# ReactiveBayes/Cortex.jl

Hardware: AMD Instinct MI355X
Metric: edge-message updates/sec per sweep, 10M-edge Gaussian grid (higher is better)
Workload: dtype f64; 1 GPU; C4: ONE 1415x1415 2-D Gaussian grid loopy BP; 10005465 bipartite edges, 16006480 owned directed message updates + 2002225 marginals per sweep; whole job 16006480 updates per sweep; schedule=fused, partition=1 row blocks, seed=1234

## Files before the change

### cortex.jl_amd/_lib.py

```python
from __future__ import annotations

import ctypes as C
import os

HERE = os.path.dirname(os.path.abspath(__file__))
LIB_PATH = os.environ.get("CORTEX_HIP_LIB", os.path.join(HERE, "libcortex_hip.so"))

ABI_VERSION = 9
OK = 0
ERR_INVALID_ARGUMENT, ERR_NOT_FOUND, ERR_UNSUPPORTED, ERR_STATE, ERR_DEVICE, ERR_NO_DEVICE, ERR_OUT_OF_MEMORY = (
    -1, -2, -3, -4, -5, -6, -7)
TO_FACTOR, TO_VARIABLE = 1, 2
ITEM_MESSAGE_TO_FACTOR, ITEM_MESSAGE_TO_VARIABLE, ITEM_INDIVIDUAL_MARGINAL = 1, 2, 4
ITEM_PRODUCT_OF_MESSAGES, ITEM_JOINT_MARGINAL = 8, 16
FORM_MOMENT, FORM_POINT, FORM_NATURAL, FORM_MEAN_PRECISION, FORM_GAMMA = 0, 1, 2, 3, 4
FACTOR_OPAQUE, FACTOR_GAUSS_ADDITIVE, FACTOR_GAUSS_LINEAR, FACTOR_NORMAL_PRECISION, FACTOR_BERNOULLI, FACTOR_GAUSS_LINEAR_N = 0, 1, 2, 3, 4, 5
NPARAM = 4
ROLE_OUT, ROLE_IN, ROLE_PRECISION = 0, 1, 2
SCHED_FLOODING, SCHED_FUSED, SCHED_CHAIN_SCAN, SCHED_TREE, SCHED_REFERENCE = 0, 1, 2, 3, 4
FAMILY_GAUSSIAN, FAMILY_NATURAL2, FAMILY_VMP_MEAN_FIELD, FAMILY_VMP_STRUCTURED = 0, 1, 2, 3
VMP_ALL_NORMAL, VMP_ALL_PRECISION = -1, -2
WIRE_WEAK, WIRE_INTERMEDIATE, WIRE_NO_LISTEN, WIRE_DEFAULT_VARIABLE, WIRE_LINK = 1, 2, 4, 8, 16
KERNEL_VAR_TO_FACTOR, KERNEL_FACTOR_TO_VAR, KERNEL_FUSED, KERNEL_BATCH, KERNEL_BIG_VAR = 0, 1, 2, 3, 4
KERNEL_HALO_BEGIN, KERNEL_HALO_END = 5, 6
# ... 52 lines not shown
    "cx_ref_trace": (_i32, [_vp, _i64, C.POINTER(Item), _pi64]),
    "cx_residual": (_i32, [_vp, _pd]),
    "cx_message_health": (_i32, [_vp, _pi64]),
    "cx_log_evidence": (_i32, [_vp, _pd, _pi64]),
    "cx_graph_components": (_i32, [_vp, _i64, _pi64, _pi64, _pi64]),
    "cx_log_evidence_components": (_i32, [_vp, _i64, _pd, _pi64, _pi64, _pi64]),
    "cx_log_evidence_mfma": (_i32, [_vp, _pd, _pi64]),
    "cx_factor_beliefs": (_i32, [_vp, _i64, _pi64, _pd]),
    "cx_factor_statistics": (_i32, [_vp, _i64, _pi64, _pi64, _i64, _pd, _pi64]),
    "cx_factor_beliefs_mfma": (_i32, [_vp, _i64, _pi64, _pd]),
    "cx_factor_statistics_mfma": (_i32, [_vp, _i64, _pi64, _pi64, _i64, _pd, _pi64]),
    "cx_sample_posterior": (_i32, [_vp, _i64, C.c_uint64, _pd, _i64, _pi64, _pd, _pi64]),
    "cx_linear_moments": (_i32, [_vp, _i64, _pi64, _pi64, _pd, _pd, _pd, _pi64]),
    "cx_predictive": (_i32, [_vp, _i32, _i64, _pi64, _pd, _pd, _pi64]),
    "cx_predictive_rows": (_i32, [_vp, _i64, _pi64, _pi64]),
    "cx_predictive_mfma": (_i32, [_vp, _i32, _i64, _pi64, _pd, _pd, _pi64]),
    "cx_predictive_rows_mfma": (_i32, [_vp, _i64, _pi64, _pi64]),
    "cx_causal_marginals": (_i32, [_vp, _i32, _i32, _i64, _pi64, _pd, _pi64]),
    "cx_causal_marginals_mfma": (_i32, [_vp, _i32, _i32, _i64, _pi64, _pd, _pi64]),
    "cx_sample_posterior_mfma": (_i32, [_vp, _i64, C.c_uint64, _pd, _i64, _pi64, _pd, _pi64]),
    "cx_set_factor_offsets": (_i32, [_vp, _i64, _pi64, _pd]),
    "cx_halo_configure": (_i32, [_vp, _i64, _pi64, _pi64, _i64, _pi64, _pi64]),
    "cx_halo_buffers": (_i32, [_vp, C.POINTER(_vp), _pi64, C.POINTER(_vp), _pi64]),
    "cx_halo_set_buffers": (_i32, [_vp, _vp, _vp]),
    "cx_sweep_begin": (_i32, [_vp]),
    "cx_sweep_main": (_i32, [_vp]),
    "cx_sweep_end": (_i32, [_vp]),
    "cx_comm_unique_id": (_i32, [_vp]),
    "cx_comm_init": (_i32, [_vp, _i32, _i32, _vp]),
    "cx_halo_peers": (_i32, [_vp, _i32, _pi32, _pi64, _pi64, _pi64, _pi64]),
    "cx_sweep_exchange": (_i32, [_vp, _i32]),
    "cx_sweep_until": (_i32, [_vp, _dbl, _i32, _i32, _pi32, _pd]),
    "cx_halo_configure_state": (_i32, [_vp, _i64, _pi64, _pi64, _i64, _pi64, _pi64]),
    "cx_halo_set_layers": (_i32, [_vp, _i64, _pi64, _pi32, _i32]),
    "cx_halo_state_pack": (_i32, [_vp]),
    "cx_halo_state_unpack": (_i32, [_vp]),
    "cx_halo_state_exchange": (_i32, [_vp]),
    "cx_halo_exchange_sweep": (_i32, [_vp, _i32]),
    "cx_halo_ipc_alloc": (_i32, [_vp, C.c_char_p, C.POINTER(C.c_void_p), _pi64]),
    "cx_halo_ipc_connect": (_i32, [_vp, _i32, C.c_char_p, C.c_void_p, _i32, _i64, _i64]),
    "cx_halo_ipc_exchange": (_i32, [_vp]),
    "cx_halo_ipc_exchange_sweep": (_i32, [_vp, _i32]),
    "cx_halo_ipc_batch": (_i32, [_vp, _i32]),
    "cx_halo_ipc_set_fused": (_i32, [_vp, _i32]),
    "cx_halo_ipc_push": (_i32, [_vp]),
    "cx_halo_ipc_unpack": (_i32, [_vp]),
    "cx_halo_ipc_status": (_i32, [_vp, _pi32, _pi64]),
    "cx_halo_ipc_set_timeout": (_i32, [_vp, C.c_double]),
    "cx_chain_block_maps": (_i32, [_vp, _pd, _pd, _pd, _pd, _pi64, _pi64, _pi64]),
    "cx_chain_plan_stats": (_i32, [_vp, _pi64]),
    "cx_chain_scan_stats": (_i32, [_vp, _pi64]),
    "cx_sweep_stats": (_i32, [_vp, _pi64]),
    "cx_sweep_deep_stats": (_i32, [_vp, _pi64]),
    "cx_tree_plan_stats": (_i32, [_vp, _pi64]),
    "cx_tree_heavy_path_stats": (_i32, [_vp, _pi64]),
    "cx_set_marginals": (_i32, [_vp, _i64, _pi64, _i32, _pd]),
    "cx_update_marginals": (_i32, [_vp, _i64, _pi64]),
    "cx_state_bytes": (_i32, [_vp, _pi64]),
    "cx_state_export": (_i32, [_vp, _vp, C.c_int64]),
    "cx_state_import": (_i32, [_vp, _vp, C.c_int64]),
    "cx_profile_enable": (_i32, [_vp, _i32]),
    "cx_profile_read": (_i32, [_vp, _i32, _pd, _pi64]),
    "cx_kernel_name": (C.c_char_p, [_i32]),
}

def item_range(lo: int, hi: int) -> int:
    return (int(lo) << 32) | int(hi)


_lib = None


class CortexHipError(RuntimeError):

    def __init__(self, code: int, message: str):
        super().__init__(f"cortex_hip status {code}: {message}")
        self.code = code
        self.message = message


def load():
    global _lib
    if _lib is not None:
        return _lib
    if not os.path.exists(LIB_PATH):
        raise ImportError(
            f"{LIB_PATH} is missing: build it with `python -m cortex.jl_amd.build` (hipcc --offload-arch=gfx950); "
            "there is no CPU fallback for the device path")
    lib = C.CDLL(LIB_PATH)
    for name, (res, args) in SIGNATURES.items():
        fn = getattr(lib, name)
        fn.restype = res
        fn.argtypes = args
    if lib.cx_version() != ABI_VERSION:
        raise ImportError(f"libcortex_hip.so ABI {lib.cx_version()} != binding ABI {ABI_VERSION}")
    _lib = lib
    return lib
```

### cortex.jl_amd/csrc/cx_api_sweep.hip

```cpp

#include "cx_host.h"
#include "cx_chains.h"
#include "cx_tree_plan.h"
#include "cx_lattice_deep.h"

using namespace cxh;

namespace cxh {

int32_t ensure_v2f(cx_handle *h) {
    if (!h->v2f_stale) return CX_OK;
    const double2 *src = h->d_f2v_alt ? h->d_f2v_alt : h->d_f2v;
    cx::launch_var_to_factor(h, src, false);
    cx::launch_big_var_to_factor(h, src, false);
    CX_HIP(h, hipGetLastError());
    h->v2f_stale = false;
    return CX_OK;
}

int32_t build_chains(cx_handle *h) {
    if (!h->chains_dirty) return CX_OK;
    if (h->cfg.dim > 1) { int32_t rc0 = mv_ensure_chain_msgs(h); if (rc0 != CX_OK) return rc0; }
    try {
        cx::chains::Out co;
// ... 243 lines not shown
                if (pi >= 0) (void)cx::chain64_tree_sweep(h, pi);
            } else if (kind == 0) {
                if (idx == h->tree_hp_marginal_stage && h->cfg.compute_marginals_in_sweep == 0) continue;
                const int64_t n = h->tree_stage_off[idx + 1] - h->tree_stage_off[idx];
                if (n > 0 && h->cfg.dim > 1) cx::mv_launch_batch(h, h->d_tree_rec + 5 * h->tree_stage_off[idx], n);
                else if (n > 0) cx::launch_batch(h, h->d_tree_rec + 5 * h->tree_stage_off[idx], n);
            } else if (h->cfg.dim > 1) {
                const int64_t l0 = h->tree_hp_link_off[idx];
                cx::mvc_launch_scan_range(h, h->tree_hp_npos, h->tree_hp_pos_off[idx + 1], l0, h->tree_hp_link_off[idx + 1] - l0, h->tree_hp_K[idx],
                                          kind == 1 ? h->d_chain_skip1 : h->d_tree_skip1_down, kind == 2);
            } else if (kind == 3) {
                const int64_t l0 = h->tree_hp_link_off[idx];
                cx::launch_kary_link_params(h, l0, h->tree_hp_link_off[idx + 1] - l0, h->d_tree_a ? h->d_tree_a : h->d_a, h->d_tree_b ? h->d_tree_b : h->d_b);
            } else {
                const int64_t p0 = h->tree_hp_pos_off[idx], l0 = h->tree_hp_link_off[idx];
                cx::launch_chain_scan_range(h, h->d_f2v, p0, h->tree_hp_pos_off[idx + 1] - p0, l0, h->tree_hp_link_off[idx + 1] - l0,
                                            kind == 1 ? h->d_chain_skip1 : h->d_tree_skip1_down, kind == 2);
            }
        }
        return;
    }
    size_t ns = h->tree_stage_off.empty() ? 0 : h->tree_stage_off.size() - 1;
    if (ns > 0 && h->cfg.compute_marginals_in_sweep == 0 && !cx::is_mfma_dim(h->cfg.dim)) ns--;
    static const bool runs = [] { const char *e = std::getenv("CX_TREE_RUNS"); return !(e && e[0] == '0'); }();
    for (size_t s = 0; s < ns;) {
        const int64_t n = h->tree_stage_off[s + 1] - h->tree_stage_off[s], nk = h->tree_kary_off[s + 1] - h->tree_kary_off[s];
        if (cx::is_mfma_dim(h->cfg.dim)) {
            const int64_t np = h->tree_pre_off[s + 1] - h->tree_pre_off[s];
            if (np > 0) cx::mv64_launch_v2f(h, (int)np, h->d_tree_pre_slots + h->tree_pre_off[s], h->d_tree_pre_vars + h->tree_pre_off[s], h->d_mv_f2v);
            if (n > 0) cx::mv64_launch_rule(h, (int)n, h->d_tree_rec + 8 * h->tree_stage_off[s], h->d_mv_f2v, h->d_mv_f2v, CX_KERNEL_BATCH);
            s++; continue;
        }
        if (h->cfg.dim > 1) { if (n > 0) cx::mv_launch_batch(h, h->d_tree_rec + 5 * h->tree_stage_off[s], n); s++; continue; }
        size_t e = s;
        while (runs && e < ns && h->tree_stage_off[e + 1] - h->tree_stage_off[e] <= 1024) e++;
        if (e >= s + 2) { cx::launch_batch_run(h, h->d_tree_rec, h->d_tree_stage_off, (int)s, (int)e); s = e; continue; }
        if (n > 0) cx::launch_batch(h, h->d_tree_rec + 5 * h->tree_stage_off[s], n);
        if (nk > 0) cx::launch_kary_items(h, h->d_tree_kary + h->tree_kary_off[s], nk);
        s++;
    }
}

int32_t tree_sweep(cx_handle *h) {
    static const bool graphs = [] { const char *e = std::getenv("CX_TREE_GRAPH"); return !(e && e[0] == '0'); }();
    cx::GraphExec &g = h->tree_graph;
    if (graphs && !h->profiling) {
        if (!g && !g.failed()) (void)capture(h, g, [h] { tree_issue(h); });
        if (g && launch(h, g)) return CX_OK;
    }
    tree_issue(h);
    return CX_OK;
}

constexpr int kDeepMax = 4, kDeepDefault = 4, kDeepMinSweeps = 16;
static int deep_depth_of_call(int32_t n_sweeps) {
    if (n_sweeps < kDeepMinSweeps) return 2;
    const char *e = std::getenv("CX_SWEEP_DEPTH");
    const int d = e ? std::atoi(e) : kDeepDefault;
    return d >= 2 && d <= kDeepMax ? d : kDeepDefault;
}

static int32_t pairs_allowed(cx_handle *h, int32_t n_sweeps, bool last_marg_only, bool *yes) {
    *yes = false;
    const char *e = std::getenv("CX_SWEEP_PAIRS");
    if (e && e[0] == '0') return CX_OK;
    if (n_sweeps < 3 || h->pair_H == 0 || h->cfg.dim != 1 || h->cfg.family != CX_FAMILY_GAUSSIAN || h->cfg.schedule != CX_SCHED_FUSED) return CX_OK;
    if (h->damping != 0.0 || h->any_linear || h->n_kary > 0 || !h->big_vars.empty() || h->halo_state || !h->recv_slots.empty() || !h->send_slots.empty() ||
        h->halo_depth > 0 || h->run_excl_lo <= h->run_excl_hi || h->cfg.materialize_messages_to_factor != 0 || h->profiling || h->d_q_gamma) return CX_OK;
    if (!(last_marg_only || h->cfg.compute_marginals_in_sweep == 0)) return CX_OK;
    if (h->pair_check_due || (!h->pair_inputs_ok && h->sweeps_done >= h->pair_check_at)) {
        h->pair_inputs_ok = true;
        for (int64_t v = 0; v < h->nv && h->pair_inputs_ok; v++)
            if ((h->vinfo[v] & (cx::kClamped | cx::kGhost)) || (h->vinfo[v] & cx::kDegMask) == cx::kBigDeg) h->pair_inputs_ok = false;
        if (h->pair_inputs_ok) {
            unsigned flag = 1;
            CX_HIP(h, hipMemsetAsync(h->d_pair_flag, 0, sizeof(unsigned), h->stream));
            cx::launch_pair_check(h, h->d_f2v, h->d_f2v_alt, h->d_pair_flag);
            CX_HIP(h, hipMemcpyAsync(&flag, h->d_pair_flag, sizeof(unsigned), hipMemcpyDeviceToHost, h->stream));
            CX_HIP(h, hipStreamSynchronize(h->stream));
            h->pair_inputs_ok = flag == 0;
        }
        h->pair_check_due = false;
        if (!h->pair_inputs_ok) h->pair_check_at = h->sweeps_done + 16;
    }
    if (!h->pair_inputs_ok) return CX_OK;
    if (h->pair_rows == 0) {
        const char *re = std::getenv("CX_PAIR_ROWS");
        cx::lattice::Plan pl;
        pl.H = h->pair_H; pl.W = h->pair_W; pl.block_cols = h->pair_block_cols;
        h->pair_rows = re && std::atoi(re) >= 1 ? std::atoi(re) : cx::lattice::choose_rows(pl, cx::pair_capacity_blocks(h));
        const char *de = std::getenv("CX_DEEP_ROWS");
        for (int d = 3; d <= kDeepMax; d++)
            h->deep_rows[d] = de && std::atoi(de) >= 1 ? std::atoi(de) : cx::lattice::deep::choose_rows_packed(pl, cx::deep_capacity_blocks(h, d), d);
    }
    *yes = true;
    return CX_OK;
}

void sweep_main(cx_handle *h, bool skip_ghosts) {
    const bool marg = h->cfg.compute_marginals_in_sweep != 0 && !h->run_skip_marg;
    if (h->cfg.schedule == CX_SCHED_CHAIN_SCAN) {
        if (!h->chain_covers_all) cx::launch_factor_to_var(h, h->d_v2f, h->d_f2v);
        const bool fast = h->chain_covers_all && h->big_vars.empty() && h->cfg.materialize_messages_to_factor == 0 && !h->offchain_marg_dirty;
        const int form = marg ? (h->d_split_mean ? 3 : (h->cfg.family == CX_FAMILY_NATURAL2 ? 2 : 1)) : 0;
        h->split_marg_written = fast && form == 3;
        cx::launch_chain_scan(h, h->d_f2v, h->chain_covers_all, fast ? form : 0, h->chain_v2f_from_scan);
        if (fast && marg) {
// ... 83 lines not shown
        double2 sf, sl;
        CX_HIP(h, hipMemcpyAsync(&sf, h->d_chain_side, 16, hipMemcpyDeviceToHost, h->stream));
        CX_HIP(h, hipMemcpyAsync(&sl, h->d_chain_side + (h->chain_npos - 1), 16, hipMemcpyDeviceToHost, h->stream));
        int32_t pv[2] = {0, 0};
        CX_HIP(h, hipMemcpyAsync(&pv[0], h->d_chain_pos_var, 4, hipMemcpyDeviceToHost, h->stream));
        CX_HIP(h, hipMemcpyAsync(&pv[1], h->d_chain_pos_var + (h->chain_npos - 1), 4, hipMemcpyDeviceToHost, h->stream));
        CX_HIP(h, hipStreamSynchronize(h->stream));
        for (int dir = 0; dir < 2; dir++) {
            HLin t{1.0, 0.0, 0.0, 1.0, 0.0, 0.0, 0, 0};
            for (int64_t i = 0; i < ntiles; i++) t = (i == 0) ? tot[(size_t)dir * (ntiles + 1)] : hlin_compose(t, tot[(size_t)dir * (ntiles + 1) + i]);
            double *o = dir == 0 ? fwd6 : bwd6;
            o[0] = t.e; o[1] = t.f; o[2] = t.g; o[3] = t.A; o[4] = t.B; o[5] = t.C;
        }
        side_first2[0] = sf.x; side_first2[1] = sf.y; side_last2[0] = sl.x; side_last2[1] = sl.y;
        if (first_variable_id) *first_variable_id = h->var_ids[pv[0]];
        if (last_variable_id) *last_variable_id = h->var_ids[pv[1]];
        if (n_links) *n_links = h->chain_nlinks;
        return CX_OK;
    } catch (const std::bad_alloc &) { return fail(h, CX_ERR_OUT_OF_MEMORY, "cx_chain_block_maps: host allocation failed"); }
}

int32_t cx_tree_plan_stats(const cx_handle *h, int64_t *out8) {
    CX_REQUIRE(const_cast<cx_handle *>(h), h && out8, CX_ERR_INVALID_ARGUMENT, "cx_tree_plan_stats: null argument");
    for (int i = 0; i < 8; i++) out8[i] = h->tree_dirty ? 0 : h->tree_stats[i];
    return CX_OK;
}

int32_t cx_tree_heavy_path_stats(const cx_handle *h, int64_t *out4) {
    CX_REQUIRE(const_cast<cx_handle *>(h), h && out4, CX_ERR_INVALID_ARGUMENT, "cx_tree_heavy_path_stats: null argument");
    for (int i = 0; i < 4; i++) out4[i] = (h->tree_dirty || !h->tree_hp) ? 0 : h->tree_hp_stats[i];
    return CX_OK;
}

int32_t cx_chain_plan_stats(const cx_handle *h, int64_t *out8) {
    if (!h || !out8) return CX_ERR_INVALID_ARGUMENT;
    cx::chain64_stats(h, out8);
    return CX_OK;
}

int32_t cx_sweep_stats(const cx_handle *h, int64_t *out4) {
    if (!h || !out4) return CX_ERR_INVALID_ARGUMENT;
    out4[0] = h->partner_run_entries; out4[1] = h->partner_run_fallback; out4[2] = h->sweeps_without_marginals; out4[3] = h->pair_launches;
    return CX_OK;
}

int32_t cx_sweep_deep_stats(const cx_handle *h, int64_t *out4) {
    if (!h || !out4) return CX_ERR_INVALID_ARGUMENT;
    const int d = h->pair_H ? h->deep_depth : 0;
    out4[0] = h->deep_launches[3]; out4[1] = h->deep_launches[4]; out4[2] = d;
    out4[3] = d == 0 ? 0 : d == 2 ? h->pair_rows : h->deep_rows[d];
    return CX_OK;
}

int32_t cx_chain_scan_stats(const cx_handle *h, int64_t *out4) {
    if (!h || !out4) return CX_ERR_INVALID_ARGUMENT;
    out4[0] = h->chain_onepass_state; out4[1] = h->chain_onepass_launches; out4[2] = h->batch_graph_launches; out4[3] = 0;
    return CX_OK;
}

int32_t cx_set_damping(cx_handle *h, double lambda) {
    CX_NOT_VMP(h, "cx_set_damping");
    CX_REQUIRE(h, h, CX_ERR_INVALID_ARGUMENT, "null handle");
    CX_REQUIRE(h, lambda >= 0.0 && lambda < 1.0, CX_ERR_INVALID_ARGUMENT, "cx_set_damping: 0 <= lambda < 1");
    CX_REQUIRE(h, lambda == 0.0 || h->cfg.schedule == CX_SCHED_FUSED || h->cfg.schedule == CX_SCHED_FLOODING, CX_ERR_UNSUPPORTED,
               "cx_set_damping: the fused and flooding schedules iterate to a fixed point and can be damped; the chain-scan, tree and reference-order schedules are exact or sequential passes");
    CX_REQUIRE(h, lambda == 0.0 || h->halo_state || (h->send_slots.empty() && h->recv_slots.empty()), CX_ERR_UNSUPPORTED,
               "cx_set_damping: not with per-sweep message halos (cx_halo_configure); state halos (cx_halo_configure_state) run plain sweeps and are damped like them");
    CX_HIP(h, hipStreamSynchronize(h->stream));
    h->damping = lambda;
    batch_graph_drop(h);
    return CX_OK;
}

int32_t cx_sweep(cx_handle *h, int32_t n_sweeps) {
    CX_NOT_VMP(h, "cx_sweep");
    CX_REQUIRE(h, h && h->has_graph, CX_ERR_STATE, "cx_sweep: no graph");
    CX_REQUIRE(h, n_sweeps >= 0, CX_ERR_INVALID_ARGUMENT, "cx_sweep: n_sweeps < 0");
    if (h->cfg.dim > 1) return mv_sweep(h, n_sweeps);
    CX_REQUIRE(h, h->halo_state || h->chain_partition || h->cfg.schedule == CX_SCHED_TREE || (h->recv_slots.empty() && h->send_slots.empty()), CX_ERR_STATE,
               "cx_sweep: this handle holds a partition (halo configured): use cx_sweep_begin / _main / _end");
    if (h->cfg.schedule == CX_SCHED_CHAIN_SCAN) { int32_t rc = build_chains(h); if (rc != CX_OK) return rc; }
    { int32_t rc = cx::kary_upload(h); if (rc != CX_OK) return rc; }
    if (h->cfg.schedule == CX_SCHED_REFERENCE) {
        CX_REQUIRE(h, h->recv_slots.empty() && h->send_slots.empty(), CX_ERR_UNSUPPORTED, "cx_sweep: the reference-order schedule is not partitioned");
        return ref_sweep_all(h, n_sweeps);
    }
    if (h->cfg.schedule == CX_SCHED_TREE) {
        int32_t rc = build_tree(h);
        if (rc != CX_OK) return rc;
        for (int32_t s = 0; s < n_sweeps; s++) { const int32_t rt = tree_sweep(h); if (rt != CX_OK) return rt; h->sweeps_done++; }
        h->v2f_stale = false;
        CX_HIP(h, hipGetLastError());
        return CX_OK;
    }
    const char *bg_env = std::getenv("CX_HALO_GRAPH");
    const bool batch_graphs = bg_env && bg_env[0] == '1';
    cx_handle::BatchGraph *bg = nullptr;
    if (batch_graphs && n_sweeps >= 4 && h->halo_state && h->halo_depth > 0 && h->cfg.schedule == CX_SCHED_FUSED && h->big_vars.empty() && h->n_kary == 0 &&
        !h->profiling && h->cfg.materialize_messages_to_factor == 0) {
        uint64_t key = 0x9e3779b97f4a7c15ull;
        for (uint64_t x : {(uint64_t)h->sweeps_since_exchange, (uint64_t)n_sweeps, (uint64_t)(uintptr_t)h->d_f2v.get(), (uint64_t)(uintptr_t)h->d_f2v_alt.get(), h->batch_epoch, (uint64_t)(uintptr_t)h->stream})
            key = (key ^ x) * 0xbf58476d1ce4e5b9ull + (key >> 29);
        for (auto &g : h->batch_graph) if (g.key == key) bg = &g;
        if (!bg) {
            bg = h->batch_graph[0].seen <= h->batch_graph[1].seen ? &h->batch_graph[0] : &h->batch_graph[1];
            *bg = cx_handle::BatchGraph();
// ... 124 lines not shown
```

### cortex.jl_amd/csrc/cx_internal.h

```cpp
#pragma once

#include <hip/hip_runtime.h>

#include <cstdint>
#include <map>
#include <memory>
#include <tuple>
#include <type_traits>
#include <string>
#include <vector>

#include "cortex_hip.h"
#include "cx_const.h"

struct cx_handle;

namespace cx {

struct ProfileRec {
    int kernel;
    hipEvent_t start, stop;
};

template <class T>
// ... 62 lines not shown
            (void)hipGetLastError();
            if (p) (void)hipHostFree(p);
            return false;
        }
        host = (volatile unsigned *)p; dev = (unsigned *)d; *host = 0;
        return true;
    }
};

template <class T> struct Deleter { void operator()(T *p) const; };
struct RefSched;
namespace ev { struct Cache; }
namespace evm { struct Cache; }
namespace lm { struct Cache; }
namespace fs { struct Cache; }
namespace sp { struct Plan; }
namespace pr { struct Plan; }
namespace prm { struct Plan; }
namespace cm { struct Plan; }
namespace cmm { struct Plan; }
namespace spm { struct Plan; }

}

namespace cx {

struct DevState {
    OwnedStream capture_stream;
    GraphExec tree_graph;
    struct BatchGraph { uint64_t key = 0; GraphExec graph; int seen = 0; };
    BatchGraph batch_graph[2];
    std::unique_ptr<RefSched, Deleter<RefSched>> ref;

    DevBuf<int32_t> d_slice_off, d_partner, d_vbase, d_var_deg;
    DevBuf<int32_t> d_big, d_big_slots, d_big_slot_var;
    DevBuf<double2> d_big_tmp;
    DevBuf<uint8_t> d_vinfo;
    DevBuf<double> d_q, d_a, d_b;
    DevBuf<double> d_sq, d_sa, d_sb;
    DevBuf<double2> d_f2v, d_v2f, d_marg;
    DevBuf<double2> d_f2v_alt;
    DevBuf<double2> d_prev;
    DevBuf<double> d_scratch;
    int sweep_max_w = 0;
    DevBuf<int16_t> d_partner16;
    DevBuf<int32_t> d_partner_runs;
    DevBuf<char> d_stage;
    int32_t pair_H = 0, pair_W = 0, pair_block_cols = 0, pair_rows = 0;
    std::string pair_refused;
    HostWord pair_abort;
    DevBuf<unsigned> d_pair_flag;
    bool pair_check_due = true, pair_inputs_ok = false;
    int64_t pair_check_at = 0, pair_launches = 0;
    int32_t deep_rows[5] = {0, 0, 0, 0, 0}, deep_depth = 0;
    int64_t deep_launches[5] = {0, 0, 0, 0, 0};

    int64_t n_kary = 0;
    std::vector<int32_t> kary_slot, slot_kary;
    std::vector<int32_t> kary_pset;
    DevBuf<int32_t> d_kary_pset, d_kary_v2f_slots, d_kary_v2f_vars;
    DevBuf<double> d_kary_aq;
    int64_t n_kary_v2f = 0, kary_aq_sets = 0;
    std::vector<double> kary_coef, kary_qb;
    DevBuf<int32_t> d_kary_slot, d_slot_kary;
    DevBuf<double> d_kary_coef, d_kary_qb;
    bool kary_dirty = true;

    DevBuf<int32_t> d_spdir;
    DevBuf<double> d_ptab;
    DevBuf<double> d_zero_msg;
    DevBuf<double> d_ptab_bt;
    int64_t ptab_sets = 0, ptab_bt_sets = 0;
    DevBuf<double> d_mv_f2v, d_mv_f2v_alt, d_mv_v2f, d_mv_marg, d_mv_prev;
    int mv_max_deg = 0;
    DevBuf<double> d_off_b, d_off_g;
    DevBuf<int32_t> d_off_rt;
    bool work64_dirty = true, point64_dirty = true;
    DevBuf<int32_t> d_point64_slots;
    DevBuf<int32_t> d_rule64_rec;
    int64_t n_pre64 = 0;
    DevBuf<int32_t> d_pre64_slots, d_pre64_vars, d_tree_pre_slots, d_tree_pre_vars;

    bool chains_dirty = true, tree_dirty = true;
    DevBuf<int32_t> d_tree_rec, d_tree_kary;
    DevBuf<int64_t> d_tree_stage_off;
    bool tree_hp = false;
    DevBuf<int32_t> d_tree_skip1_down;
    DevBuf<double> d_tree_a, d_tree_b;

    DevBuf<int32_t> d_chain_pos_var, d_chain_skip0, d_chain_skip1;
    DevBuf<int32_t> d_chain_link_pos, d_chain_from, d_chain_to;
    DevBuf<int32_t> d_chain_leaf_from;
    int64_t chain_nleaf = 0;
    DevBuf<uint8_t> d_chain_head_fwd, d_chain_head_bwd;
    DevBuf<double2> d_chain_side;
    DevBuf<char> d_chain_totals;
    DevBuf<int32_t> d_chain_tab_fwd, d_chain_tab_bwd;
    DevBuf<double> d_mvc_side, d_mvc_totals;
    DevBuf<int32_t> d_mvc_var_link;
    DevBuf<double> d_mvc_side_l, d_mvc_alpha, d_mvc_gamma, d_mvc_prefix, d_mvc_wave_carry, d_mvc_block;

    DevBuf<int32_t> d_send_slots, d_recv_slots, d_send_vars;
    DevBuf<double2> d_send_buf, d_recv_buf;

    struct SetMemo { uint64_t key = 0, used = 0; int32_t direction = 0; std::vector<int64_t> var_ids, fac_ids, edges; std::vector<int32_t> idx, vars; };
    std::vector<SetMemo> set_memos;

    std::map<std::tuple<int32_t, int32_t, int32_t>, int32_t> prod_index;
// ... 280 lines not shown
```

### cortex.jl_amd/csrc/cx_lattice_deep.h

```cpp
#pragma once

#include "cx_lattice_plan.h"

namespace cx {
namespace lattice {
namespace deep {

constexpr int kMinDepth = 2, kMaxDepth = 4;

CX_LAT_HD int strip_cols(int K) { return 64 - 2 * (K - 1); }
CX_LAT_HD int lane_col(int strip, int lane, int K) { return strip * strip_cols(K) - (K - 1) + lane; }
CX_LAT_HD bool lane_owned(int lane, int col, int W, int K) { return lane >= K - 1 && lane <= 64 - K && col < W; }
CX_LAT_HD bool lane_valid_at_level(int lane, int col, int W, int j) { return lane >= j - 1 && lane <= 64 - j && col >= 0 && col < W; }
CX_LAT_HD int row_lo(int r0, int K, int j) { return r0 - (K - j) > 0 ? r0 - (K - j) : 0; }
CX_LAT_HD int row_hi(int r1, int H, int K, int j) { return r1 + (K - j) < H ? r1 + (K - j) : H; }
CX_LAT_HD bool row_valid_at_level(int r, int r0, int r1, int H, int K, int j) { return r >= row_lo(r0, K, j) && r < row_hi(r1, H, K, j); }
CX_LAT_HD int load_lo(int r0, int K) { return row_lo(r0, K, 1); }
CX_LAT_HD int load_hi(int r1, int H, int K) { return row_hi(r1, H, K, 1); }

CX_LAT_HD bool strip_interior(int strip, int W, int K) { return lane_col(strip, 0, K) >= 1 && lane_col(strip, 63, K) <= W - 2; }
CX_LAT_HD bool segment_interior(int r0, int r1, int H, int K) { return r0 - (K - 1) >= 1 && r1 + (K - 1) - 1 <= H - 2; }

constexpr int kWaveGeneral = 0, kWaveInterior = 1, kWaveColumnEdge = 2;
CX_LAT_HD bool column_edge(int strip, int r0, int r1, int H, int W, int K) { return segment_interior(r0, r1, H, K) && !strip_interior(strip, W, K); }
CX_LAT_HD int wave_class(int strip, int r0, int r1, int H, int W, int K) {
    if (!segment_interior(r0, r1, H, K)) return kWaveGeneral;
    return strip_interior(strip, W, K) ? kWaveInterior : kWaveColumnEdge;
}

CX_LAT_HD int32_t strips(int W, int K) { return (W + strip_cols(K) - 1) / strip_cols(K); }
inline int32_t block_cols(int W, int K) { return (strips(W, K) + kStripsPerBlock - 1) / kStripsPerBlock; }

CX_LAT_HD bool packed_wave(int slab, int w, int W, int nseg, int K, int *strip, int *seg) {
    const int full = strips(W, K) / kStripsPerBlock, s = strips(W, K) - full * kStripsPerBlock;
    if (slab < full * nseg) {
        const int bc = slab / nseg;
        *strip = bc * kStripsPerBlock + w; *seg = slab - bc * nseg;
        return true;
    }
    if (s == 0) return false;
    const int per = kStripsPerBlock / s, seg0 = (slab - full * nseg) * per;
    *strip = full * kStripsPerBlock + w % s; *seg = seg0 + w / s;
    return w / s < per && *seg < nseg;
}
CX_LAT_HD int32_t packed_blocks(int W, int nseg, int K) {
    const int full = strips(W, K) / kStripsPerBlock, s = strips(W, K) - full * kStripsPerBlock;
    if (s == 0) return full * nseg;
    const int per = kStripsPerBlock / s;
    return full * nseg + (nseg + per - 1) / per;
}
inline int min_rows(int K) { return 4 * (K - 1); }

inline int choose_rows(const Plan &p, int64_t capacity_blocks, int K) {
    const int64_t seg_max = std::max<int64_t>(1, capacity_blocks / std::max<int32_t>(1, block_cols(p.W, K)));
    const int64_t R = (p.H + seg_max - 1) / seg_max;
    return (int)std::min<int64_t>(kMaxRows, std::max<int64_t>(min_rows(K), R));
}

inline int choose_rows_packed(const Plan &p, int64_t capacity_blocks, int K) {
    for (int R = min_rows(K); R < kMaxRows; R++)
        if (packed_blocks(p.W, n_segments(p, R), K) <= capacity_blocks) return R;
// ... 24 lines not shown
```

### cortex.jl_amd/csrc/cx_sweep_deep.hip

```cpp

#include "cx_scalar_core.h"
#include "cx_lattice_deep.h"

namespace cx {

namespace {

typedef double dd2v __attribute__((ext_vector_type(2)));
__device__ __forceinline__ double2 deep_load_stream(const double2 *p) {
    const dd2v v = __builtin_nontemporal_load((const dd2v *)p);
    return make_double2(v.x, v.y);
}
__device__ __forceinline__ int deep_slab(int b, int nb) {
    const int xcd = b & 7, q = nb >> 3, r = nb & 7;
    return (xcd < r ? xcd * (q + 1) : r * (q + 1) + (xcd - r) * q) + (b >> 3);
}
__device__ __forceinline__ double2 dsel2(bool c, double2 a, double2 b) { return make_double2(c ? a.x : b.x, c ? a.y : b.y); }
__device__ __forceinline__ int ishift_up(int x) { return __builtin_amdgcn_update_dpp(0, x, 0x138 , 0xf, 0xf, false); }
__device__ __forceinline__ int ishift_down(int x) { return __builtin_amdgcn_update_dpp(0, x, 0x130 , 0xf, 0xf, false); }
__device__ __forceinline__ double dshift_up(double x) { return __hiloint2double(ishift_up(__double2hiint(x)), ishift_up(__double2loint(x))); }
__device__ __forceinline__ double dshift_down(double x) { return __hiloint2double(ishift_down(__double2hiint(x)), ishift_down(__double2loint(x))); }
__device__ __forceinline__ double2 dshfl_up2(double2 a) { return make_double2(dshift_up(a.x), dshift_up(a.y)); }
__device__ __forceinline__ double2 dshfl_down2(double2 a) { return make_double2(dshift_down(a.x), dshift_down(a.y)); }

// ... 45 lines not shown
    const bool colv = COLS || (c >= 0 && c < W);
    const bool hasL = COLS || (colv && c > 0), hasR = COLS || (colv && c < W - 1);
    const bool own = dp::lane_owned(lane, c, W, K) && colv;
    const bool two = hasL && hasR;
    const int offR = (COLS ? 2 : lattice::rank_right(c)) * kBlock, offU = (COLS ? 3 : lattice::rank_up(c, W)) * kBlock;
    const int offRofL = (COLS ? 2 : lattice::rank_right(c - 1)) * kBlock;
    constexpr bool EDGE = ROWS && !COLS;
    const int ldL = hasL ? lattice::rank_left() * kBlock : 0, ldR = hasR ? offR : 0, ldU = colv ? offU : 0, ldD = colv ? offU + kBlock : 0;
    bool bad = false;

    auto in_grid = [&](int r) { return (ROWS || (r >= 0 && r < H)) && colv; };
    auto load_raw = [&](int r) { return EDGE ? slice_off[(colv ? r * W + c : 0) >> kSliceShift] : in_grid(r) ? slice_off[(r * W + c) >> kSliceShift] : 0; };
    auto finish_base = [&](int r, int raw) { return EDGE ? raw + ((colv ? r * W + c : 0) & (kBlock - 1)) : in_grid(r) ? raw + ((r * W + c) & (kBlock - 1)) : 0; };
    auto zero_row = [](int base) {
        DeepRow in;
#pragma unroll
        for (int k = 0; k < 5; k++) in.x[k] = zero2();
        in.qR = 1.0; in.qD = 1.0; in.base = base;
        return in;
    };
    auto load_row = [&](int r, int base) {
        DeepRow in = zero_row(base);
        if (EDGE) {
            in.x[0] = deep_load_stream(&f2v_in[in.base]);
            in.x[1] = deep_load_stream(&f2v_in[in.base + ldL]); in.x[2] = deep_load_stream(&f2v_in[in.base + ldR]);
            in.x[3] = deep_load_stream(&f2v_in[in.base + ldU]); in.x[4] = deep_load_stream(&f2v_in[in.base + ldD]);
            in.qR = q[in.base + ldR]; in.qD = q[in.base + ldD];
        } else if (in_grid(r)) {
            const int deg = COLS ? 5 : lattice::degree(r, c, H, W);
#pragma unroll
            for (int k = 0; k < 5; k++)
                if (k < deg) in.x[k] = deep_load_stream(&f2v_in[in.base + k * kBlock]);
            if (hasR) in.qR = q[in.base + offR];
            if (ROWS || r < H - 1) in.qD = q[in.base + (ROWS ? offU + kBlock : lattice::rank_down(r, c, W) * kBlock)];
        }
        return in;
    };

    double2 P[K];
    double qR[K], qD[K + 1];
    int base[K + 1];
#pragma unroll
    for (int a = 0; a < K; a++) { P[a] = zero2(); qR[a] = 1.0; }
#pragma unroll
    for (int a = 0; a <= K; a++) { qD[a] = 1.0; base[a] = 0; }
    DeepPending pend[K + 1];
#pragma unroll
    for (int j = 0; j <= K; j++) { pend[j].L = zero2(); pend[j].R = zero2(); pend[j].U = zero2(); pend[j].carry = zero2(); }

    const int i0 = r0 - (K - 1), i1 = r1 + (K - 1) - 1;
    DeepRow nxt = zero_row(0);
    int raw_next = load_raw(i0);
    asm volatile("" : "+v"(raw_next));
    for (int i = i0 - 1; i <= i1; i++) {
        const DeepRow cur = nxt;
        const int base_next = finish_base(i + 1, raw_next);
        if (i < i1) nxt = load_row(i + 1, base_next);
        if (i + 1 < i1) raw_next = load_raw(i + 2);
        P[0] = cur.x[0]; qR[0] = cur.qR; qD[0] = cur.qD; base[0] = cur.base;
        DeepOut e;
        e.L = zero2(); e.R = zero2(); e.up = zero2(); e.down = zero2();
        if (i >= i0 && (ROWS || (i >= 0 && i < H))) {
            const bool hasU = ROWS || i > 0, hasD = ROWS || i < H - 1;
            double2 in[5], o[5];
            const double2 xu = two ? cur.x[3] : cur.x[2];
            const double2 xd = hasU ? (two ? cur.x[4] : cur.x[3]) : xu;
            in[0] = cur.x[0];
            in[1] = dsel2(hasL, cur.x[1], zero2());
            in[2] = dsel2(hasR, EDGE || hasL ? cur.x[2] : cur.x[1], zero2());
            in[3] = EDGE ? cur.x[3] : dsel2(hasU && colv, xu, zero2());
            in[4] = EDGE ? cur.x[4] : dsel2(hasD && colv, xd, zero2());
            deep_leave_one_out(in, o);
            bad = bad || deep_undefined(o, hasL, hasR, colv && hasU, colv && hasD);
            e = deep_emit(o, hasL, hasR, cur.qR, qD[1], cur.qD);
        }
#pragma unroll
        for (int j = 2; j <= K; j++) {
            const int m = i - (j - 1);
            DeepOut f;
            f.L = zero2(); f.R = zero2(); f.up = zero2(); f.down = zero2();
            int baseL = 0, baseR = 0;
            double qL = 1.0;
            if (j == K) {
                baseL = ishift_up(base[K - 1]); baseR = ishift_down(base[K - 1]);
                qL = dshift_up(qR[K - 1]);
            }
            if (ROWS ? (m >= r0 - (K - j) && m < r1 + (K - j)) : dp::row_valid_at_level(m, r0, r1, H, K, j)) {
                const bool mU = ROWS || m > 0, mD = ROWS || m < H - 1;
                double2 in[5], o[5];
                in[0] = P[j - 1]; in[1] = pend[j].L; in[2] = pend[j].R;
                in[3] = dsel2(mU, pend[j].U, zero2());
                in[4] = dsel2(mD, e.up, zero2());
                deep_leave_one_out(in, o);
                if (dp::lane_valid_at_level(lane, COLS ? 0 : c, COLS ? 1 : W, j)) bad = bad || deep_undefined(o, hasL, hasR, mU, mD);
                if (j < K) f = deep_emit(o, hasL, hasR, qR[j - 1], qD[j], qD[j - 1]);
                else if (own) {
                    if (hasL) f2v_out[baseL + offRofL] = factor_rule<kRuleAdditive>(o[1], qL, 1.0, 0.0);
                    if (hasR) f2v_out[baseR + lattice::rank_left() * kBlock] = factor_rule<kRuleAdditive>(o[2], qR[K - 1], 1.0, 0.0);
                    if (mU) f2v_out[base[K] + (ROWS ? offU + kBlock : lattice::rank_down(m - 1, c, W) * kBlock)] = factor_rule<kRuleAdditive>(o[3], qD[K], 1.0, 0.0);
                    if (mD) f2v_out[base[K - 2] + offU] = factor_rule<kRuleAdditive>(o[4], qD[K - 1], 1.0, 0.0);
                }
            }
            pend[j].L = e.L; pend[j].R = e.R; pend[j].U = pend[j].carry; pend[j].carry = e.down;
            e = f;
        }
#pragma unroll
        for (int a = K; a >= 1; a--) {
// ... 11 lines not shown

template <int K>
__global__ __launch_bounds__(kBlock) void k_sweep_deep(int H, int W, int R, int nseg, const int32_t *__restrict__ slice_off, const double *__restrict__ q,
                                                       const double2 *__restrict__ f2v_in, double2 *__restrict__ f2v_out, unsigned *__restrict__ abort_word) {
    namespace dp = lattice::deep;
    const int s = deep_slab(blockIdx.x, gridDim.x), w = __builtin_amdgcn_readfirstlane(threadIdx.x >> 6);
    int strip, seg;
    if (!dp::packed_wave(s, w, W, nseg, K, &strip, &seg)) return;
    const int r0 = seg * R, r1 = min(r0 + R, H);
#ifdef CX_DEEP_STAMPS
    const unsigned long long st_wall = wall_clock64(), st_clk = __builtin_amdgcn_s_memtime();
#endif
    int cls = dp::wave_class(strip, r0, r1, H, W, K);
#if defined(CX_DEEP_STAMPS) && CX_DEEP_STAMPS == 2
    if (cls == dp::kWaveColumnEdge) cls = dp::kWaveGeneral;
#endif
    if (cls == dp::kWaveInterior) deep_wave<K, true, true>(strip, r0, r1, H, W, slice_off, q, f2v_in, f2v_out, abort_word);
    else if (cls == dp::kWaveColumnEdge) deep_wave<K, true, false>(strip, r0, r1, H, W, slice_off, q, f2v_in, f2v_out, abort_word);
    else deep_wave<K, false, false>(strip, r0, r1, H, W, slice_off, q, f2v_in, f2v_out, abort_word);
#ifdef CX_DEEP_STAMPS
    const unsigned long long en_clk = __builtin_amdgcn_s_memtime(), en_wall = wall_clock64();
    const unsigned hw = __builtin_amdgcn_s_getreg((4 << 0) | (0 << 6) | (31 << 11));
    const unsigned xcc = __builtin_amdgcn_s_getreg((20 << 0) | (0 << 6) | (3 << 11));
    const int slot = (int)blockIdx.x * 4 + w;
    if ((threadIdx.x & 63) == 0 && slot < kDeepStampWaves) {
        unsigned long long *rec = cx_deep_stamps + (size_t)slot * 8;
        rec[0] = st_wall; rec[1] = en_wall; rec[2] = st_clk; rec[3] = en_clk;
        rec[4] = (unsigned long long)hw | (unsigned long long)xcc << 32;
        rec[5] = (unsigned long long)(unsigned)strip | (unsigned long long)(unsigned)seg << 32;
        rec[6] = 1ull + (unsigned long long)cls; rec[7] = blockIdx.x;
    }
#endif
}

#ifdef CX_DEEP_STAMPS
extern "C" __attribute__((visibility("default"))) int32_t cx_lab_deep_stamps(unsigned long long *out, int32_t max_waves) {
    const int n = max_waves < kDeepStampWaves ? max_waves : kDeepStampWaves;
    if (hipDeviceSynchronize() != hipSuccess || hipMemcpyFromSymbol(out, HIP_SYMBOL(cx_deep_stamps), (size_t)n * 64) != hipSuccess) return -1;
    static unsigned long long zeros[kDeepStampWaves * 8];
    if (hipMemcpyToSymbol(HIP_SYMBOL(cx_deep_stamps), zeros, sizeof zeros) != hipSuccess) return -1;
    return n;
}
#endif

template <int K>
static int64_t deep_capacity(const cx_handle *h) {
    int per_cu = 0, dev = h->cfg.device;
    hipDeviceProp_t prop;
    if (hipOccupancyMaxActiveBlocksPerMultiprocessor(&per_cu, k_sweep_deep<K>, kBlock, 0) != hipSuccess || per_cu <= 0) { (void)hipGetLastError(); per_cu = 2; }
    if (hipGetDeviceProperties(&prop, dev) != hipSuccess) { (void)hipGetLastError(); return (int64_t)per_cu * 256; }
    return (int64_t)per_cu * prop.multiProcessorCount;
}

int64_t deep_capacity_blocks(const cx_handle *h, int depth) { return depth == 3 ? deep_capacity<3>(h) : deep_capacity<4>(h); }

void launch_sweep_deep(cx_handle *h, int depth, const double2 *f2v_in, double2 *f2v_out) {
    const int R = h->deep_rows[depth], nseg = (h->pair_H + R - 1) / R;
    const dim3 grid((unsigned)lattice::deep::packed_blocks(h->pair_W, nseg, depth));
    if (depth == 3)
        hipLaunchKernelGGL(k_sweep_deep<3>, grid, dim3(kBlock), 0, h->stream, h->pair_H, h->pair_W, R, nseg, h->d_slice_off, h->d_q, f2v_in, f2v_out, h->pair_abort.dev);
    else
        hipLaunchKernelGGL(k_sweep_deep<4>, grid, dim3(kBlock), 0, h->stream, h->pair_H, h->pair_W, R, nseg, h->d_slice_off, h->d_q, f2v_in, f2v_out, h->pair_abort.dev);
}

}
```

### cortex.jl_amd/device.py

```python
from __future__ import annotations

import ctypes as C
from typing import Optional

import numpy as np

from . import _lib as L


def _i64(a):
    return np.ascontiguousarray(a, dtype=np.int64)


def _f64(a):
    return np.ascontiguousarray(a, dtype=np.float64)


def _p(a, ct):
    return a.ctypes.data_as(C.POINTER(ct))


class DeviceGraph:
    def __init__(self, device: int = 0, dim: int = 1, schedule: int = L.SCHED_FUSED, marginals_in_sweep: bool = True,
                 materialize_messages_to_factor: bool = False, family: int = L.FAMILY_GAUSSIAN):
# ... 55 lines not shown

    def set_factor_offsets(self, factor_ids, b):
        f = _i64(np.atleast_1d(factor_ids))
        b = _f64(b).reshape(-1, self.dim) if len(f) else _f64(np.zeros((0, self.dim)))
        if len(b) != len(f):
            raise ValueError(f"b must be [{len(f)}, {self.dim}]")
        self._check(self.lib.cx_set_factor_offsets(self.h, len(f), _p(f, C.c_int64) if len(f) else None, _p(b, C.c_double) if len(f) else None))

    def linear_factors_of_set(self, parameter_set: int):
        lin = self._factor_kind == L.FACTOR_GAUSS_LINEAR
        return self._factor_ids[lin & (self._factor_params[:, 0] == int(parameter_set))]

    def set_factor_edge_sets(self, variable_ids, factor_ids, parameter_sets):
        v, f, s = _i64(np.atleast_1d(variable_ids)), _i64(np.atleast_1d(factor_ids)), _i64(np.atleast_1d(parameter_sets))
        self._check(self.lib.cx_set_factor_edge_sets(self.h, len(v), _p(v, C.c_int64), _p(f, C.c_int64), _p(s, C.c_int64)))

    def stats(self) -> dict:
        s = L.Stats()
        self._check(self.lib.cx_graph_stats(self.h, C.byref(s)))
        return {k: getattr(s, k) for k, _ in L.Stats._fields_}

    def tree_plan_stats(self):
        out = (C.c_int64 * 8)()
        self._check(self.lib.cx_tree_plan_stats(self.h, out))
        keys = ("depth", "stages", "items", "kary_entries", "components", "messages_up", "messages_down", "marginals")
        return dict(zip(keys, [int(x) for x in out]))

    def tree_heavy_path_stats(self):
        out = (C.c_int64 * 4)()
        self._check(self.lib.cx_tree_heavy_path_stats(self.h, out))
        return dict(zip(("light_depths", "paths", "single_variables", "launches"), [int(x) for x in out]))

    def chain_plan_stats(self):
        out = (C.c_int64 * 8)()
        self._check(self.lib.cx_chain_plan_stats(self.h, out))
        keys = ("links_per_block", "fan", "levels", "potentials", "compositions", "rules", "launches", "device_bytes")
        return dict(zip(keys, (int(x) for x in out)))

    def chain_scan_stats(self):
        out = (C.c_int64 * 4)()
        self._check(self.lib.cx_chain_scan_stats(self.h, out))
        return {"state": int(out[0]), "launches": int(out[1]), "halo_batch_graph_launches": int(out[2])}

    def sweep_stats(self):
        out = (C.c_int64 * 4)()
        self._check(self.lib.cx_sweep_stats(self.h, out))
        return {"partner_run_entries": int(out[0]), "partner_run_fallback": int(out[1]), "sweeps_without_marginals": int(out[2]),
                "paired_launches": int(out[3])}

    def sweep_deep_stats(self):
        out = (C.c_int64 * 4)()
        self._check(self.lib.cx_sweep_deep_stats(self.h, out))
        return {"depth3_launches": int(out[0]), "depth4_launches": int(out[1]), "depth": int(out[2]), "rows": int(out[3])}

    def edge_index(self, variable_ids, factor_ids):
        v, f = _i64(np.atleast_1d(variable_ids)), _i64(np.atleast_1d(factor_ids))
        out = np.zeros(len(v), dtype=np.int64)
        self._check(self.lib.cx_edge_index(self.h, len(v), _p(v, C.c_int64), _p(f, C.c_int64), _p(out, C.c_int64)))
        return out

    def set_messages(self, variable_ids, factor_ids, direction: int, form: int, payload):
        v, f = _i64(np.atleast_1d(variable_ids)), _i64(np.atleast_1d(factor_ids))
        p = _f64(payload)
        need = len(v) * self.lib.cx_payload_doubles(self.dim, form)
        if p.size != need:
            raise ValueError(f"payload has {p.size} doubles, expected {need}")
        self._check(self.lib.cx_set_messages(self.h, len(v), _p(v, C.c_int64), _p(f, C.c_int64), direction, form,
                                             _p(p, C.c_double)))

    def get_messages(self, variable_ids, factor_ids, direction: int, form: int = L.FORM_MOMENT):
        v, f = _i64(np.atleast_1d(variable_ids)), _i64(np.atleast_1d(factor_ids))
        out = np.zeros((len(v), self.lib.cx_payload_doubles(self.dim, L.FORM_MOMENT)), dtype=np.float64)
        self._check(self.lib.cx_get_messages(self.h, len(v), _p(v, C.c_int64), _p(f, C.c_int64), direction, form,
                                             _p(out, C.c_double)))
        return out

    def seed_messages(self, direction: int, mean: float, variance: float):
        self._check(self.lib.cx_seed_messages(self.h, direction, float(mean), float(variance)))

    def get_marginals(self, variable_ids):
        v = _i64(np.atleast_1d(variable_ids))
        out = np.zeros((len(v), self.lib.cx_payload_doubles(self.dim, L.FORM_MOMENT)), dtype=np.float64)
        self._check(self.lib.cx_get_marginals(self.h, len(v), _p(v, C.c_int64), _p(out, C.c_double)))
        return out

    def update_batch(self, kinds, variable_ids, factor_ids):
        n = len(kinds)
        items = (L.Item * n)()
        for i in range(n):
            items[i].kind = int(kinds[i])
            items[i].variable_id = int(variable_ids[i])
            items[i].factor_id = int(factor_ids[i])
        self._check(self.lib.cx_update_batch(self.h, items, n))

    def update_batch_packed(self, records: bytes, n: int):
        if self._batch_raw is None:
            proto = C.CFUNCTYPE(C.c_int32, C.c_void_p, C.c_char_p, C.c_int64)
            self._batch_raw = proto(("cx_update_batch_async", self.lib))
        rc = self._batch_raw(self.h, records, n)
        if rc != L.OK:
            self._check(rc)

    def get_products(self, variable_ids, range_lo, range_hi, form: int = L.FORM_MOMENT):
        v = _i64(np.atleast_1d(variable_ids))
        lo = np.ascontiguousarray(np.atleast_1d(range_lo), dtype=np.int32)
        hi = np.ascontiguousarray(np.atleast_1d(range_hi), dtype=np.int32)
# ... 452 lines not shown
```

### include/cortex_hip.h

```cpp
#ifndef CORTEX_HIP_H
#define CORTEX_HIP_H

#include <stdint.h>

#ifdef __cplusplus
extern "C" {
#endif

#define CX_ABI_VERSION 9

#define CX_OK 0
#define CX_ERR_INVALID_ARGUMENT (-1)
#define CX_ERR_NOT_FOUND (-2)
#define CX_ERR_UNSUPPORTED (-3)
#define CX_ERR_STATE (-4)
#define CX_ERR_DEVICE (-5)
#define CX_ERR_NO_DEVICE (-6)
#define CX_ERR_OUT_OF_MEMORY (-7)

#define CX_TO_FACTOR 1
#define CX_TO_VARIABLE 2

#define CX_ITEM_MESSAGE_TO_FACTOR 1
#define CX_ITEM_MESSAGE_TO_VARIABLE 2
// ... 58 lines not shown
    int64_t n_slices, n_big_variables, n_slots;
    int64_t device_bytes;
    int64_t sweeps_done;
} cx_stats;

int32_t cx_version(void);
int32_t cx_create(const cx_config *config, cx_handle **out);
int32_t cx_destroy(cx_handle *h);
const char *cx_last_error(const cx_handle *h);
int32_t cx_sync(cx_handle *h);
int32_t cx_set_stream(cx_handle *h, void *hip_stream);

int32_t cx_graph_create(cx_handle *h, int64_t n_edges, const int64_t *edge_var, const int64_t *edge_fac,
                        const int32_t *edge_role, int64_t n_factors, const int64_t *factor_ids,
                        const int32_t *factor_kind, const double *factor_params);
int32_t cx_set_factor_matrices(cx_handle *h, int64_t parameter_set, const double *A, const double *Q);
int32_t cx_set_factor_coefficients(cx_handle *h, int64_t n, const int64_t *variable_ids, const int64_t *factor_ids, const double *a);
int32_t cx_set_factor_edge_sets(cx_handle *h, int64_t n, const int64_t *variable_ids, const int64_t *factor_ids, const int64_t *parameter_sets);
int32_t cx_graph_stats(const cx_handle *h, cx_stats *out);
int32_t cx_edge_index(const cx_handle *h, int64_t n, const int64_t *variable_ids, const int64_t *factor_ids,
                      int64_t *out_edge);

int64_t cx_payload_doubles(int32_t dim, int32_t form);
int32_t cx_set_messages(cx_handle *h, int64_t n, const int64_t *variable_ids, const int64_t *factor_ids,
                        int32_t direction, int32_t form, const double *payload);
int32_t cx_get_messages(cx_handle *h, int64_t n, const int64_t *variable_ids, const int64_t *factor_ids,
                        int32_t direction, int32_t form, double *out);
#define CX_VMP_ALL_NORMAL (-1)
#define CX_VMP_ALL_PRECISION (-2)
int32_t cx_set_marginals(cx_handle *h, int64_t n, const int64_t *variable_ids, int32_t form, const double *payload);
int32_t cx_update_marginals(cx_handle *h, int64_t n, const int64_t *variable_ids);

int32_t cx_seed_messages(cx_handle *h, int32_t direction, double mean, double variance);
int32_t cx_get_marginals(cx_handle *h, int64_t n, const int64_t *variable_ids, double *out);

int32_t cx_update_batch(cx_handle *h, const cx_item *items, int64_t n);
int32_t cx_update_batch_async(cx_handle *h, const cx_item *items, int64_t n);
int32_t cx_get_products(cx_handle *h, int64_t n, const int64_t *variable_ids, const int32_t *range_lo, const int32_t *range_hi,
                        int32_t form, double *out);
int32_t cx_get_joint_marginals(cx_handle *h, int64_t n, const int64_t *factor_ids, double *out);
int32_t cx_sweep(cx_handle *h, int32_t n_sweeps);
int32_t cx_set_damping(cx_handle *h, double lambda);
int32_t cx_sweep_for(cx_handle *h, int64_t n, const int64_t *variable_ids);
#define CX_WIRE_WEAK 1
#define CX_WIRE_INTERMEDIATE 2
#define CX_WIRE_NO_LISTEN 4
#define CX_WIRE_DEFAULT_VARIABLE 8
#define CX_WIRE_LINK 16
int32_t cx_graph_wire(cx_handle *h, int64_t n, const cx_item *signals, const cx_item *dependencies, const int32_t *flags);
int32_t cx_ref_plan_stats(const cx_handle *h, int64_t *out8);
int32_t cx_chain_scan_stats(const cx_handle *h, int64_t *out4);
int32_t cx_sweep_stats(const cx_handle *h, int64_t *out4);
int32_t cx_sweep_deep_stats(const cx_handle *h, int64_t *out4);
int32_t cx_cluster_stats(const cx_handle *h, int64_t *out4);
int32_t cx_ref_trace(const cx_handle *h, int64_t capacity, cx_item *out, int64_t *n_executions);
int32_t cx_residual(cx_handle *h, double *out_max_abs_delta);
int32_t cx_sweep_until(cx_handle *h, double tol, int32_t max_sweeps, int32_t check_every, int32_t *sweeps_run, double *residual);

int32_t cx_halo_configure(cx_handle *h, int64_t n_send, const int64_t *send_variable_ids,
                          const int64_t *send_factor_ids, int64_t n_recv, const int64_t *recv_variable_ids,
                          const int64_t *recv_factor_ids);
int32_t cx_halo_buffers(cx_handle *h, void **send_device_ptr, int64_t *send_bytes, void **recv_device_ptr,
                        int64_t *recv_bytes);
int32_t cx_halo_set_buffers(cx_handle *h, void *send_device_ptr, void *recv_device_ptr);
int32_t cx_sweep_begin(cx_handle *h);
int32_t cx_sweep_main(cx_handle *h);
int32_t cx_sweep_end(cx_handle *h);

int32_t cx_comm_unique_id(void *out128);
int32_t cx_comm_init(cx_handle *h, int32_t world, int32_t rank, const void *id128);
int32_t cx_halo_peers(cx_handle *h, int32_t n_peers, const int32_t *peer_rank, const int64_t *send_offset,
                      const int64_t *send_count, const int64_t *recv_offset, const int64_t *recv_count);
int32_t cx_sweep_exchange(cx_handle *h, int32_t n_sweeps);

int32_t cx_halo_configure_state(cx_handle *h, int64_t n_send, const int64_t *send_var, const int64_t *send_fac,
                                int64_t n_recv, const int64_t *recv_var, const int64_t *recv_fac);
int32_t cx_halo_set_layers(cx_handle *h, int64_t n, const int64_t *variable_ids, const int32_t *layer, int32_t depth);
int32_t cx_halo_state_pack(cx_handle *h);
int32_t cx_halo_state_unpack(cx_handle *h);
int32_t cx_halo_state_exchange(cx_handle *h);
int32_t cx_halo_exchange_sweep(cx_handle *h, int32_t n_sweeps);
int32_t cx_halo_ipc_alloc(cx_handle *h, void *handle64, void **local_base, int64_t *area_bytes);
int32_t cx_halo_ipc_connect(cx_handle *h, int32_t peer_index, const void *handle64, void *same_process_base, int32_t remote_entry,
                            int64_t remote_recv_off, int64_t remote_area_bytes);
int32_t cx_halo_ipc_push(cx_handle *h);
int32_t cx_halo_ipc_unpack(cx_handle *h);
int32_t cx_halo_ipc_exchange(cx_handle *h);
int32_t cx_halo_ipc_exchange_sweep(cx_handle *h, int32_t n_sweeps);
int32_t cx_halo_ipc_batch(cx_handle *h, int32_t n_sweeps);
int32_t cx_halo_ipc_set_fused(cx_handle *h, int32_t on);
int32_t cx_halo_ipc_status(cx_handle *h, int32_t *timed_out, int64_t *exchanges);
int32_t cx_halo_ipc_set_timeout(cx_handle *h, double seconds);

int32_t cx_chain_block_maps(cx_handle *h, double *forward6, double *backward6, double *side_first2, double *side_last2,
                            int64_t *first_variable_id, int64_t *last_variable_id, int64_t *n_links);

int32_t cx_chain_plan_stats(const cx_handle *h, int64_t *out8);

int32_t cx_tree_plan_stats(const cx_handle *h, int64_t *out8);
int32_t cx_tree_heavy_path_stats(const cx_handle *h, int64_t *out4);

int32_t cx_message_health(cx_handle *h, int64_t *out4);

int32_t cx_log_evidence(cx_handle *h, double *value, int64_t *counts4);

int32_t cx_factor_beliefs(cx_handle *h, int64_t n, const int64_t *factor_ids, double *out);
// ... 59 lines not shown
```

Measured before the change: 762.8 billion edge-message updates/s.

## Extend temporal-blocked deep sweep to depths 5 and 6 and stagger wave priority

Raises the maximum fused sweep depth (multiple BP sweeps per kernel launch over a row strip) from 4 to 6 and makes 5 the default, adding template instantiations and launch dispatch for K=5 and K=6. Each launch then covers more sweeps, cutting global memory traffic and launch count per sweep, at the cost of narrower useful strip columns (64-2(K-1)) and more redundant halo recomputation. It also sets wave priority high at the start of each segment loop and lowers it in quarters, so waves that are further along yield to ones that are behind. A stats query for per-depth launch counts is added.

```diff
diff --git a/cortex.jl_amd/_lib.py b/cortex.jl_amd/_lib.py
--- a/cortex.jl_amd/_lib.py
+++ b/cortex.jl_amd/_lib.py
@@ -128,6 +128,7 @@
     "cx_chain_scan_stats": (_i32, [_vp, _pi64]),
     "cx_sweep_stats": (_i32, [_vp, _pi64]),
     "cx_sweep_deep_stats": (_i32, [_vp, _pi64]),
+    "cx_sweep_deep_launches": (_i32, [_vp, _pi64]),
     "cx_tree_plan_stats": (_i32, [_vp, _pi64]),
     "cx_tree_heavy_path_stats": (_i32, [_vp, _pi64]),
     "cx_set_marginals": (_i32, [_vp, _i64, _pi64, _i32, _pd]),
diff --git a/cortex.jl_amd/csrc/cx_api_sweep.hip b/cortex.jl_amd/csrc/cx_api_sweep.hip
--- a/cortex.jl_amd/csrc/cx_api_sweep.hip
+++ b/cortex.jl_amd/csrc/cx_api_sweep.hip
@@ -319,7 +319,9 @@
     return CX_OK;
 }
 
-constexpr int kDeepMax = 4, kDeepDefault = 4, kDeepMinSweeps = 16;
+constexpr int kDeepMax = 6, kDeepDefault = 5, kDeepMinSweeps = 16;
+static_assert(kDeepMax == cx::lattice::deep::kMaxDepth && sizeof(cx_handle::deep_rows) / sizeof(int32_t) == kDeepMax + 1 &&
+              sizeof(cx_handle::deep_launches) / sizeof(int64_t) == kDeepMax + 1, "deep_rows and deep_launches are indexed by depth");
 static int deep_depth_of_call(int32_t n_sweeps) {
     if (n_sweeps < kDeepMinSweeps) return 2;
     const char *e = std::getenv("CX_SWEEP_DEPTH");
@@ -509,6 +511,13 @@
     return CX_OK;
 }
 
+int32_t cx_sweep_deep_launches(const cx_handle *h, int64_t *out7) {
+    if (!h || !out7) return CX_ERR_INVALID_ARGUMENT;
+    out7[0] = 0; out7[1] = 0; out7[2] = h->pair_launches;
+    for (int d = 3; d <= kDeepMax; d++) out7[d] = h->deep_launches[d];
+    return CX_OK;
+}
+
 int32_t cx_chain_scan_stats(const cx_handle *h, int64_t *out4) {
     if (!h || !out4) return CX_ERR_INVALID_ARGUMENT;
     out4[0] = h->chain_onepass_state; out4[1] = h->chain_onepass_launches; out4[2] = h->batch_graph_launches; out4[3] = 0;
diff --git a/cortex.jl_amd/csrc/cx_internal.h b/cortex.jl_amd/csrc/cx_internal.h
--- a/cortex.jl_amd/csrc/cx_internal.h
+++ b/cortex.jl_amd/csrc/cx_internal.h
@@ -138,8 +138,8 @@
     DevBuf<unsigned> d_pair_flag;
     bool pair_check_due = true, pair_inputs_ok = false;
     int64_t pair_check_at = 0, pair_launches = 0;
-    int32_t deep_rows[5] = {0, 0, 0, 0, 0}, deep_depth = 0;
-    int64_t deep_launches[5] = {0, 0, 0, 0, 0};
+    int32_t deep_rows[7] = {}, deep_depth = 0;
+    int64_t deep_launches[7] = {};
 
     int64_t n_kary = 0;
     std::vector<int32_t> kary_slot, slot_kary;
diff --git a/cortex.jl_amd/csrc/cx_lattice_deep.h b/cortex.jl_amd/csrc/cx_lattice_deep.h
--- a/cortex.jl_amd/csrc/cx_lattice_deep.h
+++ b/cortex.jl_amd/csrc/cx_lattice_deep.h
@@ -6,7 +6,7 @@
 namespace lattice {
 namespace deep {
 
-constexpr int kMinDepth = 2, kMaxDepth = 4;
+constexpr int kMinDepth = 2, kMaxDepth = 6;
 
 CX_LAT_HD int strip_cols(int K) { return 64 - 2 * (K - 1); }
 CX_LAT_HD int lane_col(int strip, int lane, int K) { return strip * strip_cols(K) - (K - 1) + lane; }
diff --git a/cortex.jl_amd/csrc/cx_sweep_deep.hip b/cortex.jl_amd/csrc/cx_sweep_deep.hip
--- a/cortex.jl_amd/csrc/cx_sweep_deep.hip
+++ b/cortex.jl_amd/csrc/cx_sweep_deep.hip
@@ -121,7 +121,13 @@
     DeepRow nxt = zero_row(0);
     int raw_next = load_raw(i0);
     asm volatile("" : "+v"(raw_next));
+    const int quarter = (i1 - i0 + 2) >> 2;
+    const int p1 = i0 - 1 + quarter, p2 = p1 + quarter, p3 = p2 + quarter;
+    __builtin_amdgcn_s_setprio(3);
     for (int i = i0 - 1; i <= i1; i++) {
+        if (i == p1) __builtin_amdgcn_s_setprio(2);
+        else if (i == p2) __builtin_amdgcn_s_setprio(1);
+        else if (i == p3) __builtin_amdgcn_s_setprio(0);
         const DeepRow cur = nxt;
         const int base_next = finish_base(i + 1, raw_next);
         if (i < i1) nxt = load_row(i + 1, base_next);
@@ -239,15 +245,29 @@
     return (int64_t)per_cu * prop.multiProcessorCount;
 }
 
-int64_t deep_capacity_blocks(const cx_handle *h, int depth) { return depth == 3 ? deep_capacity<3>(h) : deep_capacity<4>(h); }
+int64_t deep_capacity_blocks(const cx_handle *h, int depth) {
+    switch (depth) {
+    case 3: return deep_capacity<3>(h);
+    case 4: return deep_capacity<4>(h);
+    case 5: return deep_capacity<5>(h);
+    default: return deep_capacity<6>(h);
+    }
+}
+
+template <int K>
+static void deep_launch(cx_handle *h, dim3 grid, int R, int nseg, const double2 *f2v_in, double2 *f2v_out) {
+    hipLaunchKernelGGL(k_sweep_deep<K>, grid, dim3(kBlock), 0, h->stream, h->pair_H, h->pair_W, R, nseg, h->d_slice_off, h->d_q, f2v_in, f2v_out, h->pair_abort.dev);
+}
 
 void launch_sweep_deep(cx_handle *h, int depth, const double2 *f2v_in, double2 *f2v_out) {
     const int R = h->deep_rows[depth], nseg = (h->pair_H + R - 1) / R;
     const dim3 grid((unsigned)lattice::deep::packed_blocks(h->pair_W, nseg, depth));
-    if (depth == 3)
-        hipLaunchKernelGGL(k_sweep_deep<3>, grid, dim3(kBlock), 0, h->stream, h->pair_H, h->pair_W, R, nseg, h->d_slice_off, h->d_q, f2v_in, f2v_out, h->pair_abort.dev);
-    else
-        hipLaunchKernelGGL(k_sweep_deep<4>, grid, dim3(kBlock), 0, h->stream, h->pair_H, h->pair_W, R, nseg, h->d_slice_off, h->d_q, f2v_in, f2v_out, h->pair_abort.dev);
-}
-
-}
+    switch (depth) {
+    case 3: deep_launch<3>(h, grid, R, nseg, f2v_in, f2v_out); break;
+    case 4: deep_launch<4>(h, grid, R, nseg, f2v_in, f2v_out); break;
+    case 5: deep_launch<5>(h, grid, R, nseg, f2v_in, f2v_out); break;
+    default: deep_launch<6>(h, grid, R, nseg, f2v_in, f2v_out); break;
+    }
+}
+
+}
diff --git a/cortex.jl_amd/device.py b/cortex.jl_amd/device.py
--- a/cortex.jl_amd/device.py
+++ b/cortex.jl_amd/device.py
@@ -131,6 +131,11 @@
         out = (C.c_int64 * 4)()
         self._check(self.lib.cx_sweep_deep_stats(self.h, out))
         return {"depth3_launches": int(out[0]), "depth4_launches": int(out[1]), "depth": int(out[2]), "rows": int(out[3])}
+
+    def sweep_deep_launches(self):
+        out = (C.c_int64 * 7)()
+        self._check(self.lib.cx_sweep_deep_launches(self.h, out))
+        return tuple(int(x) for x in out)
 
     def edge_index(self, variable_ids, factor_ids):
         v, f = _i64(np.atleast_1d(variable_ids)), _i64(np.atleast_1d(factor_ids))
diff --git a/include/cortex_hip.h b/include/cortex_hip.h
--- a/include/cortex_hip.h
+++ b/include/cortex_hip.h
@@ -134,6 +134,7 @@
 int32_t cx_chain_scan_stats(const cx_handle *h, int64_t *out4);
 int32_t cx_sweep_stats(const cx_handle *h, int64_t *out4);
 int32_t cx_sweep_deep_stats(const cx_handle *h, int64_t *out4);
+int32_t cx_sweep_deep_launches(const cx_handle *h, int64_t *out7);
 int32_t cx_cluster_stats(const cx_handle *h, int64_t *out4);
 int32_t cx_ref_trace(const cx_handle *h, int64_t capacity, cx_item *out, int64_t *n_executions);
 int32_t cx_residual(cx_handle *h, double *out_max_abs_delta);
```

New measurement: 804.8 billion edge-message updates/s (median of 6 runs). 5.5% higher.
